# chaofengc/FeMaSR

Measured on AMD Instinct MI355X. Metric: SR output megapixels/sec at x4 (128->512), higher is better.
Workload: dtype f32 (1x1 convs / nn.Linear: every fp32 operand split EXACTLY into three bf16 terms, six partial products, fp32 accumulation on the bf16 matrix pipe - closer to fp64 than the fp32 fmaf chain, bit-identical to the CPU oracle)

## Files before the change

femasr_amd/_lib.py:

```python
import ctypes
import os

_HERE = os.path.dirname(os.path.abspath(__file__))
SO_PATH = os.path.join(_HERE, 'csrc', 'libfemasr_hip.so')

c_int, c_i64, c_f32 = ctypes.c_int, ctypes.c_int64, ctypes.c_float
vp, szt = ctypes.c_void_p, ctypes.c_size_t


class FemasrError(RuntimeError):
    pass


MAX_CODEBOOKS = 3


class Config(ctypes.Structure):
    _fields_ = ([(n, ctypes.c_int32) for n in ('in_channel', 'gt_resolution', 'lq_stage', 'scale_factor', 'use_quantize',
                                               'use_residual', 'n_codebooks')] +
                [(n, ctypes.c_int32 * MAX_CODEBOOKS) for n in ('codebook_scale', 'n_e', 'e_dim')] +
                [('device', ctypes.c_int32)])


class ConvArgs(ctypes.Structure):
    _fields_ = [
        ('in_', vp), ('B', ctypes.c_int32), ('H', ctypes.c_int32), ('W', ctypes.c_int32), ('Cin', ctypes.c_int32),
        ('w', vp), ('bias', vp),
        ('Cout', ctypes.c_int32), ('ksz', ctypes.c_int32), ('stride', ctypes.c_int32), ('pad', ctypes.c_int32),
        ('up2', ctypes.c_int32), ('prologue', ctypes.c_int32),
        ('pro_a', vp), ('pro_b', vp), ('pro_c', vp),
        ('act', ctypes.c_int32),
        ('res1', vp), ('res2', vp), ('out', vp),
        ('Ho', ctypes.c_int32), ('Wo', ctypes.c_int32),
        ('w_bf16x3', vp), ('gn_part', vp), ('w_up2', vp), ('w_wino', vp), ('fast_act', ctypes.c_int32), ('in_add', vp), ('w_bf16s', vp),
    ]


ABI_VERSION = 106
PRO_NONE, PRO_GN_SILU, PRO_LN = 0, 1, 2
ACT_NONE, ACT_GELU, ACT_RELU = 0, 1, 2

SIGNATURES = {
    'femasr_last_error': (ctypes.c_char_p, []),
    'femasr_version': (c_int, []),
    'femasr_create': (c_int, [ctypes.POINTER(Config), ctypes.POINTER(vp)]),
    'femasr_destroy': (None, [vp]),
    'femasr_num_weights': (c_int, [vp]),
    'femasr_weight_info': (c_int, [vp, c_int, ctypes.POINTER(ctypes.c_char_p), ctypes.POINTER(c_i64 * 4), ctypes.POINTER(c_int)]),
    'femasr_set_weight': (c_int, [vp, ctypes.c_char_p, vp, ctypes.POINTER(c_i64), c_int]),
    'femasr_finalize_weights': (c_int, [vp]),
    'femasr_set_streams': (c_int, [vp, c_int]),
    'femasr_workspace_bytes': (c_int, [vp, c_int, c_int, c_int, c_int, ctypes.POINTER(szt)]),
    'femasr_forward_shapes': (c_int, [vp, c_int, c_int, c_int, ctypes.POINTER(c_int), ctypes.POINTER(c_int), ctypes.POINTER(c_int),
# ... 119 lines not shown
```

femasr_amd/csrc/build.py:

```python
import os
import subprocess
import sys

HERE = os.path.dirname(os.path.abspath(__file__))
SOURCES = ['kernels_conv.hip', 'kernels_gemm.hip', 'kernels_gemm_bf16.hip', 'kernels_vq.hip', 'kernels_wino.hip', 'kernels_wino_up2.hip', 'kernels_conv_bf16.hip', 'kernels_misc.hip', 'model.hip', 'lpips.hip', 'psnr_ssim.hip', 'niqe.hip']
HEADERS = ['common.h', 'conv_common.h', 'wino_common.h', 'detmath.h', '../../include/femasr_hip.h', '../../include/femasr_hip_debug.h']
SO = os.path.join(HERE, 'libfemasr_hip.so')
FLAGS = ['--offload-arch=gfx950', '-O3', '-std=c++17', '-fPIC', '-ffp-contract=off',
         '-fhip-fp32-correctly-rounded-divide-sqrt', '-Wno-unused-result']


def _stale(target, deps):
    if not os.path.exists(target):
        return True
    t = os.path.getmtime(target)
    return any(os.path.getmtime(d) > t for d in deps)


def build(force=False, verbose=True, gate='fail'):
    hipcc = os.environ.get('HIPCC', '/opt/rocm/bin/hipcc')
    hdrs = [os.path.join(HERE, h) for h in HEADERS]
    objs, jobs = [], []
    for src in SOURCES:
        s = os.path.join(HERE, src)
# ... 9 lines not shown
        raise RuntimeError(f'hipcc failed for {failed}')
    if force or _stale(SO, objs):
        cmd = [hipcc, '--offload-arch=gfx950', '-shared', '-fPIC', '-o', SO] + objs
        if verbose:
            print(' '.join(cmd), flush=True)
        subprocess.check_call(cmd)
    if gate != 'off' and os.environ.get('FEMASR_SKIP_SCRATCH_CHECK') != '1':
        sys.path.insert(0, HERE)
        import kernel_meta
        problems = []
        try:
            _, bad = kernel_meta.check()
            if bad:
                problems.append('kernels of the default schedule use (more) scratch memory:\n' + kernel_meta.table(bad) +
                                '(fix the spill, or list the instantiation in kernel_meta.py with the reason)')
            problems += kernel_meta.check_counted_waits()
        except Exception as e:
            print(f'kernel_meta: checks skipped ({type(e).__name__}: {e})', flush=True)
        if problems and gate == 'warn':
            print('WARNING: ' + '\n'.join(problems), flush=True)
        elif problems:
            os.remove(SO)
            raise RuntimeError('\n'.join(problems))
    return SO


if __name__ == '__main__':
    build(force='--force' in sys.argv)
```

femasr_amd/csrc/common.h:

```cpp
#pragma once
#include <hip/hip_runtime.h>
#include <stdint.h>
#include <stddef.h>
#include "../../include/femasr_hip_debug.h"

int femasr_set_error(int code, const char *fmt, ...);
#define FEMASR_CHECK_HIP(expr)                                                            \
    do {                                                                                  \
        hipError_t _e = (expr);                                                           \
        if (_e != hipSuccess)                                                             \
            return femasr_set_error(FEMASR_ERR_HIP, "%s failed: %s (%s:%d)", #expr,       \
                                    hipGetErrorString(_e), __FILE__, __LINE__);           \
    } while (0)
#define FEMASR_REQUIRE(cond, ...)                                                         \
    do {                                                                                  \
        if (!(cond)) return femasr_set_error(FEMASR_ERR_INVALID, __VA_ARGS__);            \
    } while (0)

inline int femasr_allow_dynamic_lds(const void *kern, unsigned long long *devs, size_t bytes)
{
    int dev = 0;
    FEMASR_CHECK_HIP(hipGetDevice(&dev));
    if (dev < 0 || dev >= 64 || !((__atomic_load_n(devs, __ATOMIC_ACQUIRE) >> dev) & 1ull)) {
        FEMASR_CHECK_HIP(hipFuncSetAttribute(kern, hipFuncAttributeMaxDynamicSharedMemorySize, (int)bytes));
// ... 23 lines not shown
}

bool femasr_gemm_eligible(const femasr_conv_args *a);
int femasr_gemm_launch(hipStream_t s, const femasr_conv_args *a, const conv_vq_epilogue *vq, int *variant_out, double *flops_out);
int femasr_gemm_variant_count();
int femasr_gemm_pick_variant(const femasr_conv_args *a, bool vq);
const char *femasr_gemm_variant_name(int v);
int femasr_repack_k1(hipStream_t s, const float *in, int O, int I, float *out);

bool femasr_gemm_bf16s_shape_ok(const femasr_conv_args *a);
bool femasr_conv3x3_bf16s_shape_ok(const femasr_conv_args *a);
int femasr_gemm_bf16s_launch(hipStream_t s, const femasr_conv_args *a, const void *w_bf16s, int *variant_out, double *flops_out);
int femasr_gemm_bf16s_variant_count();
int femasr_gemm_bf16s_pick_variant(const femasr_conv_args *a);
const char *femasr_gemm_bf16s_variant_name(int v);

constexpr int FEMASR_WINO_LOG2_TOTAL = 31, FEMASR_WINO_LOG2_IMAGE = 27;
bool femasr_conv_wino_shape_ok(const femasr_conv_args *a);
bool femasr_conv_wino_shape_ok_lim(const femasr_conv_args *a, int log2_total, int log2_image);
int femasr_conv_wino_gn_tiles(int H, int W);
int femasr_conv_wino_launch(hipStream_t s, const femasr_conv_args *a, int *variant_out, double *flops_out);
int femasr_conv_wino_variant_count();
int femasr_conv_wino_pick_variant(const femasr_conv_args *a);
const char *femasr_conv_wino_variant_name(int v);
bool femasr_conv_wino_up2_shape_ok(const femasr_conv_args *a);
bool femasr_conv_wino_up2_shape_ok_lim(const femasr_conv_args *a, int log2_total, int log2_image);
int femasr_conv_wino_up2_launch(hipStream_t s, const femasr_conv_args *a, double *flops_out);
const char *femasr_conv_wino_up2_variant_name();

bool femasr_conv_bf16x3_eligible(const femasr_conv_args *a);
// ... 18 lines not shown
```

femasr_amd/csrc/kernel_meta.py:

```python
import os
import re
import struct
import subprocess
import sys
import tempfile

HERE = os.path.dirname(os.path.abspath(__file__))
READELF = '/opt/rocm/lib/llvm/bin/llvm-readelf'
ALLOW_SCRATCH = (
    'conv3x3_halo_bf16x3_kernel',
)


def device_elf(obj_path):
    data = open(obj_path, 'rb').read()
    i = data.find(b'__CLANG_OFFLOAD_BUNDLE__')
    if i < 0:
        return None
    n = struct.unpack_from('<Q', data, i + 24)[0]
    off = i + 32
    for _ in range(n):
        o, sz, tl = struct.unpack_from('<QQQ', data, off)
        off += 24
        triple = data[off:off + tl].decode()
# ... 69 lines not shown
            return False
        for k, lim in KNOWN_SCRATCH.items():
            if k in r['name']:
                return sz > lim
        return True
    bad = [r for r in rows if over(r)]
    if verbose:
        print(table(rows))
    return rows, bad


OBJDUMP = '/opt/rocm/lib/llvm/bin/llvm-objdump'
VMEM_PREFIXES = ('global_', 'buffer_', 'scratch_', 'flat_', 'tbuffer_')
COUNTED = {'loops': 1, 'global_load_lds_dwordx4': 12, 'global_load_dwordx4': 8, 'vmcnt': {14: 2, 10: 4}}
N_GEMM_BF16S = 9


def disassemble(obj_path):
    elf = device_elf(obj_path)
    if not elf:
        return {}
    with tempfile.NamedTemporaryFile(suffix='.co') as t:
        t.write(elf)
        t.flush()
        txt = subprocess.run([OBJDUMP, '-d', t.name], capture_output=True, text=True, check=True).stdout
    out, cur = {}, None
    for line in txt.splitlines():
        m = re.match(r'^[0-9a-f]+ <(\S+)>:', line)
        if m:
            cur = out.setdefault(m.group(1), [])
# ... 15 lines not shown
        except (ValueError, IndexError):
            continue
        if simm >= 32768:
            simm -= 65536
        if simm >= 0:
            continue
        tgt = addr_index.get(a + 4 + 4 * simm)
        if tgt is None:
            continue
        if any(o.startswith('v_mfma') for _, o, _ in insts[tgt:i]):
            loops.append((tgt, i))
    return [l for l in loops if not any(m != l and l[0] <= m[0] and m[1] <= l[1] for m in loops)]


def check_counted_waits(obj=None):
    obj = obj or os.path.join(HERE, 'kernels_gemm_bf16.o')
    problems = []
    src = open(os.path.join(HERE, 'kernels_gemm_bf16.hip')).read()
    src_counts = sorted({int(v) for v in re.findall(r's_waitcnt vmcnt\((\d+)\)', src)})
    want_counts = sorted({0} | set(COUNTED['vmcnt']))
    if src_counts != want_counts:
        problems.append(f'kernels_gemm_bf16.hip waits for vmcnt {src_counts}, kernel_meta.COUNTED expects {want_counts}: update both together')
    seen = 0
    for name, insts in disassemble(obj).items():
        if 'gemm_bf16s_kernel' not in name:
            continue
        seen += 1
        want = COUNTED
        loops = mfma_loops(insts)
        if len(loops) != want['loops']:
            problems.append(f'{demangle_short(name)}: expected {want["loops"]} MFMA loop(s), found {len(loops)}')
            continue
        for lo, hi in loops:
            body = insts[lo:hi + 1]
            vmem, waits = {}, {}
            for _, op, args in body:
                if op.startswith(VMEM_PREFIXES):
                    vmem[op] = vmem.get(op, 0) + 1
                if op == 's_waitcnt':
                    for n in re.findall(r'vmcnt\((\d+)\)', args):
                        waits[int(n)] = waits.get(int(n), 0) + 1
            want_vmem = {k: v for k, v in want.items() if k not in ('vmcnt', 'loops')}
            if vmem != want_vmem:
                problems.append(f'{demangle_short(name)}: VMEM instructions in the MFMA loop {vmem}, the counted waits assume exactly {want_vmem}')
            if waits != want['vmcnt']:
                problems.append(f'{demangle_short(name)}: vmcnt waits in the MFMA loop {waits}, the source has {want["vmcnt"]}')
            if not any(op == 's_barrier' for _, op, _ in body):
                problems.append(f'{demangle_short(name)}: no s_barrier in the MFMA loop')
    if seen < N_GEMM_BF16S:
        problems.append(f'only {seen} gemm_bf16s_kernel instantiations found in {obj}')
    return problems


META = ('vgpr_count', 'agpr_count', 'sgpr_count', 'vgpr_spill_count', 'sgpr_spill_count', 'private_segment_fixed_size', 'group_segment_fixed_size')


def code_of(csrc, objs=None):
    meta = {(r['file'], r['name']): tuple(r.get(k) for k in META) for r in kernels(csrc) if objs is None or r['file'] in objs}
    return {f: {n: ([i[1:] for i in insts], meta[f, n]) for n, insts in disassemble(os.path.join(csrc, f)).items() if (f, n) in meta}
            for f in sorted({f for f, _ in meta})}


def diff(here, there, rename=()):
    ren = dict(rename)
    lines = []
# ... 8 lines not shown
if __name__ == '__main__':
    if '--diff' in sys.argv:
        pairs = [tuple(sys.argv[i + 1].split('=', 1)) for i, a in enumerate(sys.argv) if a == '--rename']
        lines = diff(code_of(HERE), code_of(sys.argv[sys.argv.index('--diff') + 1]), pairs)
        for f, n, what in lines:
            print('%-24s %-10s %s' % (f, what, n))
        print({w: sum(1 for l in lines if l[2] == w) for w in ('same', 'differs', 'only here', 'only there')})
        sys.exit(1 if any(l[2] == 'differs' for l in lines) else 0)
    rows, bad = check(verbose='--quiet' not in sys.argv)
    if '--table' in sys.argv:
        open(sys.argv[sys.argv.index('--table') + 1], 'w').write(table(rows))
    if bad:
        print('kernels of the default schedule that use scratch memory:')
        print(table(bad))
        sys.exit(1)
    probs = check_counted_waits()
    if probs:
        print('\n'.join(probs))
        sys.exit(1)
```

femasr_amd/csrc/kernels_gemm_bf16.hip:

```cpp
#include "conv_common.h"
#include "detmath.h"
#include <stdlib.h>

typedef float f32x16 __attribute__((ext_vector_type(16)));
typedef __bf16 bf16x8 __attribute__((ext_vector_type(8)));
typedef __bf16 bf16x2_t __attribute__((ext_vector_type(2)));
typedef float f32x2_t __attribute__((ext_vector_type(2)));

namespace {

struct GemmSParams {
    const float *A;
    const uint4 *W;
    const float *bias, *res1, *res2;
    float *out;
    int M, N, K, MB, NB, NT32;
    int imH, imW, Cin, tapmul;
    int imHo, imWo, stride;
};

__device__ float g_gs_zero_page[64];

constexpr int GS_A_HALF = 3 * 2 * 128;
constexpr int GS_A_BYTES = 2 * GS_A_HALF * 16;
constexpr int GS_W_STAGE = 4 * 3 * 64;
constexpr int GS_W_STAGES = 4;
constexpr int GS_LDS_BYTES = GS_A_BYTES + GS_W_STAGES * GS_W_STAGE * 16;
static_assert(4 * TSCRATCH * 4 <= GS_LDS_BYTES, "epilogue scratch overlays the main-loop buffers");

__device__ __forceinline__ unsigned cvt_pk_bf16(float a, float b)
{
    const bf16x2_t r = __builtin_convertvector(f32x2_t{a, b}, bf16x2_t);
    return __builtin_bit_cast(unsigned, r);
}

__device__ __forceinline__ void split3_pair(float a, float b, unsigned &p1, unsigned &p2, unsigned &p3)
{
    p1 = cvt_pk_bf16(a, b);
    const float ra = a - __uint_as_float(p1 << 16), rb = b - __uint_as_float(p1 & 0xffff0000u);
    p2 = cvt_pk_bf16(ra, rb);
    const float sa = ra - __uint_as_float(p2 << 16), sb = rb - __uint_as_float(p2 & 0xffff0000u);
    p3 = cvt_pk_bf16(sa, sb);
}
__device__ __forceinline__ void split3_x8(const f32x4_t &u, const f32x4_t &v, uint4 &q1, uint4 &q2, uint4 &q3)
{
    split3_pair(u[0], u[1], q1.x, q2.x, q3.x);
    split3_pair(u[2], u[3], q1.y, q2.y, q3.y);
    split3_pair(v[0], v[1], q1.z, q2.z, q3.z);
    split3_pair(v[2], v[3], q1.w, q2.w, q3.w);
}

typedef __attribute__((address_space(3))) void *lds_vptr_s;

__device__ __forceinline__ void dma3(const uint4 *w, unsigned d0)
{
    unsigned m0_keep;
    asm volatile("s_mov_b32 %0, m0\n\t"
                 "s_mov_b32 m0, %1\n\ts_nop 0\n\tglobal_load_lds_dwordx4 %4, off\n\t"
                 "s_mov_b32 m0, %2\n\ts_nop 0\n\tglobal_load_lds_dwordx4 %5, off\n\t"
                 "s_mov_b32 m0, %3\n\ts_nop 0\n\tglobal_load_lds_dwordx4 %6, off\n\t"
                 "s_mov_b32 m0, %0"
                 : "=&s"(m0_keep) : "s"(d0), "s"(d0 + 1024u), "s"(d0 + 2048u), "v"(w), "v"(w + 64), "v"(w + 128) : "memory");
}

template <int ACT, int NRES, int CONV>
__global__ __launch_bounds__(256, 2) void gemm_bf16s_kernel(const GemmSParams p)
{
    extern __shared__ __attribute__((aligned(16))) unsigned char smem_raw[];
    uint4 *S = reinterpret_cast<uint4 *>(smem_raw);

    const int t = threadIdx.x, lane = t & 63;
    const int wave = __builtin_amdgcn_readfirstlane(t >> 6);
    const int wm = wave >> 1, wn = wave & 1;
    const int L = xcd_remap(blockIdx.x, p.MB * p.NB);
    const int nb = L % p.NB, mb = L / p.NB;
    const int m0 = mb * 128, n0 = nb * 128;
    const int h = lane >> 5, c31 = lane & 31;
    const int nsteps = p.K >> 4;
// ... 323 lines not shown
{
    const int nres = (a->res1 ? 1 : 0) + (a->res2 ? 1 : 0), act = a->act == FEMASR_ACT_GELU ? 1 : 0;
    return a->ksz == 3 ? 6 + nres : 3 * act + nres;
}

int femasr_gemm_bf16s_launch(hipStream_t s, const femasr_conv_args *a, const void *w_bf16s, int *variant_out, double *flops_out)
{
    FEMASR_REQUIRE(a && a->in && w_bf16s && femasr_gemm_bf16s_shape_ok(a), "gemm_bf16s: layer is neither a 1x1 / linear layer nor a 3x3 pad-1 conv of stride 1 or 2 with Cin %% 64 == 0");
    FEMASR_REQUIRE(a->bias && a->out, "gemm_bf16s: bias/out must be set");
    FEMASR_REQUIRE(a->act == FEMASR_ACT_NONE || a->act == FEMASR_ACT_GELU, "gemm_bf16s: bad activation %d", a->act);
    const bool conv = a->ksz == 3;
    const int Ho = conv ? (a->H - 1) / a->stride + 1 : a->H, Wo = conv ? (a->W - 1) / a->stride + 1 : a->W;
    const long long M = (long long)a->B * Ho * Wo;
    FEMASR_REQUIRE(a->Ho == Ho && a->Wo == Wo, "gemm_bf16s: Ho/Wo mismatch");
    FEMASR_REQUIRE(M > 0 && M < (1ll << 31) - 256, "gemm_bf16s: bad row count");
    GemmSParams p{};
    p.A = a->in; p.W = (const uint4 *)w_bf16s; p.bias = a->bias; p.res1 = a->res1; p.res2 = a->res2; p.out = a->out;
    p.M = (int)M; p.N = a->Cout; p.K = conv ? 9 * a->Cin : a->Cin;
    p.imH = a->H; p.imW = a->W; p.imHo = Ho; p.imWo = Wo; p.stride = a->stride; p.Cin = a->Cin; p.tapmul = ((1 << 20) + (a->Cin >> 5) - 1) / (a->Cin >> 5);
    p.NT32 = (p.N + 31) / 32;
    p.MB = (p.M + 127) / 128; p.NB = (p.N + 127) / 128;
    const int vi = femasr_gemm_bf16s_pick_variant(a);
    GSVariant &v = g_gsv[vi];
    FEMASR_CHECK(femasr_allow_dynamic_lds((const void *)v.kern, &v.attr_devs, GS_LDS_BYTES));
    hipLaunchKernelGGL(v.kern, dim3((unsigned)(p.MB * p.NB)), dim3(256), (size_t)GS_LDS_BYTES, s, p);
    FEMASR_CHECK_HIP(hipGetLastError());
    if (variant_out) *variant_out = vi;
    if (flops_out) *flops_out = 2.0 * (double)M * (double)a->Cout * (double)p.K;
    return FEMASR_OK;
}
```

femasr_amd/csrc/kernels_misc.hip:

```cpp
#include "common.h"
#include "detmath.h"
#include <stdlib.h>
#include <string.h>
#include <type_traits>

namespace {

__device__ __forceinline__ float4 ld4(const float *p) { return *reinterpret_cast<const float4 *>(p); }

__device__ __forceinline__ int xcd_remap_misc(int bid, int nblk)
{
    const int q = nblk >> 3, r = nblk & 7, xcd = bid & 7, within = bid >> 3;
    return (xcd < r ? xcd * (q + 1) : r * (q + 1) + (xcd - r) * q) + within;
}

__global__ void pad_nchw_to_nhwc_kernel(const float *__restrict__ in, int B, int C, int H, int W, int Hp, int Wp,
                                        float *__restrict__ out, size_t total)
{
    for (size_t i = blockIdx.x * (size_t)blockDim.x + threadIdx.x; i < total; i += (size_t)gridDim.x * blockDim.x) {
        const int c = (int)(i % C);
        size_t r = i / C;
        const int x = (int)(r % Wp);
        r /= Wp;
        const int y = (int)(r % Hp);
// ... 220 lines not shown
{
    const int c4n = C >> 2;
    for (size_t i = blockIdx.x * (size_t)blockDim.x + threadIdx.x; i < total4; i += (size_t)gridDim.x * blockDim.x) {
        const int c4 = (int)(i % c4n);
        const size_t n = (i / c4n) / (size_t)hw;
        const float4 v = ld4(x + 4 * i), ga = ld4(a + n * C + 4 * c4), gb = ld4(b + n * C + 4 * c4);
        float4 o;
        o.x = det_silu(__builtin_fmaf(v.x, ga.x, gb.x));
        o.y = det_silu(__builtin_fmaf(v.y, ga.y, gb.y));
        o.z = det_silu(__builtin_fmaf(v.z, ga.z, gb.z));
        o.w = det_silu(__builtin_fmaf(v.w, ga.w, gb.w));
        *reinterpret_cast<float4 *>(y + 4 * i) = o;
    }
}

__device__ __forceinline__ float wave_tree_sum(float p)
{
#pragma unroll
    for (int s = 32; s >= 1; s >>= 1) p = p + __shfl_xor(p, s, 64);
    return p;
}

__global__ void ln_stats_kernel(const float *__restrict__ x, long long rows, float eps, float *__restrict__ stats)
{
    const long long row = (long long)blockIdx.x * (blockDim.x >> 6) + (threadIdx.x >> 6);
    if (row >= rows) return;
    const int lane = threadIdx.x & 63;
    const float4 v = ld4(x + row * 256 + lane * 4);
    float s = v.x;
    s = s + v.y;
    s = s + v.z;
    s = s + v.w;
    const float mean = wave_tree_sum(s) * (1.0f / 256.0f);
    float d = v.x - mean;
    float q = d * d;
    d = v.y - mean;
    q = __builtin_fmaf(d, d, q);
    d = v.z - mean;
    q = __builtin_fmaf(d, d, q);
    d = v.w - mean;
    q = __builtin_fmaf(d, d, q);
    const float var = wave_tree_sum(q) * (1.0f / 256.0f);
    if (lane == 0) {
        stats[2 * row] = mean;
        stats[2 * row + 1] = 1.0f / sqrtf(var + eps);
    }
}

__global__ void layernorm_kernel(const float *__restrict__ x, long long rows, const float *__restrict__ gamma,
                                 const float *__restrict__ beta, float eps, float *__restrict__ y)
{
    const long long row = (long long)blockIdx.x * (blockDim.x >> 6) + (threadIdx.x >> 6);
    if (row >= rows) return;
    const int lane = threadIdx.x & 63;
    const float4 v = ld4(x + row * 256 + lane * 4);
    float s = v.x;
    s = s + v.y;
    s = s + v.z;
    s = s + v.w;
    const float mean = wave_tree_sum(s) * (1.0f / 256.0f);
    float d = v.x - mean;
    float q = d * d;
    d = v.y - mean;
    q = __builtin_fmaf(d, d, q);
    d = v.z - mean;
    q = __builtin_fmaf(d, d, q);
    d = v.w - mean;
    q = __builtin_fmaf(d, d, q);
    const float var = wave_tree_sum(q) * (1.0f / 256.0f);
    const float rstd = 1.0f / sqrtf(var + eps);
    const float4 g = ld4(gamma + lane * 4), b = ld4(beta + lane * 4);
    float4 o;
    o.x = __builtin_fmaf((v.x - mean) * rstd, g.x, b.x);
    o.y = __builtin_fmaf((v.y - mean) * rstd, g.y, b.y);
    o.z = __builtin_fmaf((v.z - mean) * rstd, g.z, b.z);
    o.w = __builtin_fmaf((v.w - mean) * rstd, g.w, b.w);
    *reinterpret_cast<float4 *>(y + row * 256 + lane * 4) = o;
}

constexpr int ATT_HD = 32, ATT_N = 64;
typedef float att_f32x16 __attribute__((ext_vector_type(16)));

template <int UNITS>
__global__ __launch_bounds__(64, 2) void window_attention_reg_kernel(const float *__restrict__ qkv, int B, int H, int W, int C,
                                                                     int heads, int shift, const float *__restrict__ table,
                                                                     float *__restrict__ out, int total)
{
    __shared__ float Ts[UNITS][232];
    const int lane = threadIdx.x, c = lane & 31, hf = lane >> 5;
    const int nwx = W >> 3, nwy = H >> 3;
    struct Unit { int h, wx, wy, n; };
    auto unit_of = [&](int bid) {
// ... 819 lines not shown

const char *femasr_conv_form_variant_name(ConvForm f, int v)
{
    switch (f) {
    case CONV_BF16X3: return femasr_conv_bf16x3_variant_name(v);
    case CONV_WINO: return femasr_conv_wino_variant_name(v);
    case CONV_WINO_UP2: return femasr_conv_wino_up2_variant_name();
    case CONV_SPLIT: return femasr_gemm_bf16s_variant_name(v);
    default: return femasr_conv_variant_name(v);
    }
}

int femasr_conv_form_launch(hipStream_t s, ConvForm f, const femasr_conv_args *a, int *slot_out, double *flops_out)
{
    int v = 0, r;
    switch (f) {
    case CONV_BF16X3: r = femasr_conv_bf16x3_launch(s, a, &v, flops_out); break;
    case CONV_WINO: r = femasr_conv_wino_launch(s, a, &v, flops_out); break;
    case CONV_WINO_UP2: r = femasr_conv_wino_up2_launch(s, a, flops_out); break;
    case CONV_SPLIT: r = femasr_gemm_bf16s_launch(s, a, a->w_bf16s, &v, flops_out); break;
    default: r = femasr_conv2d_launch(s, a, nullptr, &v, flops_out); break;
    }
    for (int g = 0; g < f; ++g) v += femasr_conv_form_variant_count((ConvForm)g);
    if (slot_out) *slot_out = v;
    return r;
}

static ConvForm conv2d_form(const femasr_conv_args *a)
{
    return !a ? CONV_DIRECT : a->w_bf16s ? CONV_SPLIT : a->w_bf16x3 ? CONV_BF16X3 : !a->w_wino ? CONV_DIRECT : a->up2 ? CONV_WINO_UP2 : CONV_WINO;
// ... 38 lines not shown
```

femasr_amd/csrc/model.hip:

```cpp
#include <stdarg.h>
#include <stdio.h>
#include <stdlib.h>
#include <string.h>

#include <algorithm>
#include <array>
#include <map>
#include <string>
#include <vector>

#include "common.h"

static thread_local char g_err[1024] = "";

int femasr_set_error(int code, const char *fmt, ...)
{
    va_list ap;
    va_start(ap, fmt);
    vsnprintf(g_err, sizeof(g_err), fmt, ap);
    va_end(ap);
    return code;
}

namespace {
// ... 763 lines not shown
    return run_tail(c, x, feats, false, false, nullptr, out_nchw, hq << h->max_depth, wq << h->max_depth);
}

int check_ready(const femasr_handle *h)
{
    FEMASR_REQUIRE(h, "null handle");
    if (!h->finalized) return femasr_set_error(FEMASR_ERR_WEIGHT, "weights not finalized: call femasr_set_weight for every key, then femasr_finalize_weights");
    return FEMASR_OK;
}

}

extern "C" {

const char *femasr_last_error(void) { return g_err; }
int femasr_version(void) { return 106; }

int femasr_create(const femasr_config *cfg, femasr_handle **out)
{
    FEMASR_REQUIRE(cfg && out, "create: null argument");
    FEMASR_REQUIRE(cfg->in_channel == 3, "create: in_channel must be 3");
    FEMASR_REQUIRE(cfg->n_codebooks >= 1 && cfg->n_codebooks <= FEMASR_MAX_CODEBOOKS, "create: n_codebooks must be 1..%d", FEMASR_MAX_CODEBOOKS);
    for (int q = 0; q < cfg->n_codebooks; ++q) {
        FEMASR_REQUIRE(cfg->n_e[q] > 0 && cfg->n_e[q] % 128 == 0 && cfg->e_dim[q] > 0 && cfg->e_dim[q] % 32 == 0,
                       "create: codebook %dx%d unsupported (n_e %% 128, e_dim %% 32)", cfg->n_e[q], cfg->e_dim[q]);
        FEMASR_REQUIRE(cfg->codebook_scale[q] > 0 && cfg->gt_resolution % cfg->codebook_scale[q] == 0, "create: bad codebook scale");
        FEMASR_REQUIRE(q == 0 || cfg->codebook_scale[q] > cfg->codebook_scale[q - 1], "create: codebook scales must ascend");
    }
    femasr_handle *h = new femasr_handle();
    h->cfg = *cfg;
    h->scale = cfg->lq_stage ? cfg->scale_factor : 1;
// ... 392 lines not shown
```

include/femasr_hip.h:

```cpp
#ifndef FEMASR_HIP_H
#define FEMASR_HIP_H

#include <stddef.h>
#include <stdint.h>

#ifdef __cplusplus
extern "C" {
#endif

typedef enum {
    FEMASR_OK = 0,
    FEMASR_ERR_INVALID = -1,
    FEMASR_ERR_HIP = -2,
    FEMASR_ERR_WEIGHT = -3,
    FEMASR_ERR_WORKSPACE = -4
} femasr_status;

typedef struct femasr_handle femasr_handle;

#define FEMASR_MAX_CODEBOOKS 3
typedef struct {
    int32_t in_channel;
    int32_t gt_resolution;
    int32_t lq_stage;
// ... 62 lines not shown
    const float *pro_a;
    const float *pro_b;
    const float *pro_c;
    int32_t act;
    const float *res1;
    const float *res2;
    float *out;
    int32_t Ho, Wo;
    const void *w_bf16x3;
    double *gn_part;
    const float *w_up2;
    const float *w_wino;
    int32_t fast_act;
    const float *in_add;
    const void *w_bf16s;
} femasr_conv_args;
int femasr_conv2d(void *stream, const femasr_conv_args *a);

size_t femasr_gn_scratch_bytes(int B, int H, int W, int C, int G);
int femasr_gn_coeffs(void *stream, const float *x, int B, int H, int W, int C, int G,
                     const float *gamma, const float *beta, float eps, float *a, float *b, void *scratch);
int femasr_gn_coeffs_from_partials(void *stream, const double *part, int B, int tiles, int H, int W, int C, int G,
                                   const float *gamma, const float *beta, float eps, float *a, float *b);
int femasr_gn_silu_apply(void *stream, const float *x, int B, int H, int W, int C, const float *a, const float *b, float *y);
int femasr_ln_stats(void *stream, const float *x, int64_t rows, int C, float eps, float *stats);
int femasr_layernorm(void *stream, const float *x, int64_t rows, int C, const float *gamma, const float *beta,
                     float eps, float *y);
int femasr_window_attention(void *stream, const float *qkv, int B, int H, int W, int C, int heads, int shift,
                            const float *table, float *out);
int femasr_vq(void *stream, const float *z, int64_t M, int D, const float *cb, const float *cbT,
// ... 84 lines not shown
```

Measured before the change: 67.91.

## Add row-owning 1x1 Cout=256 bf16x3 GEMM kernel with optional fused LayerNorm output

Adds a new GEMM kernel for 1x1 layers with 256 output channels and no activation. Each 64-row block computes all 256 columns, so a whole output row lives in one block and the epilogue can apply bias and residuals and optionally write a LayerNorm of the row. The existing bf16s launcher now routes eligible layers to this kernel. This is meant to get better A-tile reuse and to open the door to fusing the following LayerNorm. The model code shown never sets ln_out, so the LN fusion is plumbing only. The new kernel uses a smaller M tile, so the block count and occupancy trade-offs change.

```diff
diff --git a/femasr_amd/_lib.py b/femasr_amd/_lib.py
--- a/femasr_amd/_lib.py
+++ b/femasr_amd/_lib.py
@@ -33,10 +33,11 @@
         ('res1', vp), ('res2', vp), ('out', vp),
         ('Ho', ctypes.c_int32), ('Wo', ctypes.c_int32),
         ('w_bf16x3', vp), ('gn_part', vp), ('w_up2', vp), ('w_wino', vp), ('fast_act', ctypes.c_int32), ('in_add', vp), ('w_bf16s', vp),
+        ('ln_gamma', vp), ('ln_beta', vp), ('ln_eps', c_f32), ('ln_out', vp),
     ]
 
 
-ABI_VERSION = 106
+ABI_VERSION = 107
 PRO_NONE, PRO_GN_SILU, PRO_LN = 0, 1, 2
 ACT_NONE, ACT_GELU, ACT_RELU = 0, 1, 2
 
diff --git a/femasr_amd/csrc/build.py b/femasr_amd/csrc/build.py
--- a/femasr_amd/csrc/build.py
+++ b/femasr_amd/csrc/build.py
@@ -3,8 +3,8 @@
 import sys
 
 HERE = os.path.dirname(os.path.abspath(__file__))
-SOURCES = ['kernels_conv.hip', 'kernels_gemm.hip', 'kernels_gemm_bf16.hip', 'kernels_vq.hip', 'kernels_wino.hip', 'kernels_wino_up2.hip', 'kernels_conv_bf16.hip', 'kernels_misc.hip', 'model.hip', 'lpips.hip', 'psnr_ssim.hip', 'niqe.hip']
-HEADERS = ['common.h', 'conv_common.h', 'wino_common.h', 'detmath.h', '../../include/femasr_hip.h', '../../include/femasr_hip_debug.h']
+SOURCES = ['kernels_conv.hip', 'kernels_gemm.hip', 'kernels_gemm_bf16.hip', 'kernels_gemm_bf16_rows.hip', 'kernels_vq.hip', 'kernels_wino.hip', 'kernels_wino_up2.hip', 'kernels_conv_bf16.hip', 'kernels_misc.hip', 'model.hip', 'lpips.hip', 'psnr_ssim.hip', 'niqe.hip']
+HEADERS = ['common.h', 'conv_common.h', 'wino_common.h', 'detmath.h', 'split_bf16.h', 'layernorm_row.h', '../../include/femasr_hip.h', '../../include/femasr_hip_debug.h']
 SO = os.path.join(HERE, 'libfemasr_hip.so')
 FLAGS = ['--offload-arch=gfx950', '-O3', '-std=c++17', '-fPIC', '-ffp-contract=off',
          '-fhip-fp32-correctly-rounded-divide-sqrt', '-Wno-unused-result']
@@ -47,7 +47,7 @@
             if bad:
                 problems.append('kernels of the default schedule use (more) scratch memory:\n' + kernel_meta.table(bad) +
                                 '(fix the spill, or list the instantiation in kernel_meta.py with the reason)')
-            problems += kernel_meta.check_counted_waits()
+            problems += kernel_meta.check_counted_waits() + kernel_meta.check_counted_waits_rows()
         except Exception as e:
             print(f'kernel_meta: checks skipped ({type(e).__name__}: {e})', flush=True)
         if problems and gate == 'warn':
diff --git a/femasr_amd/csrc/common.h b/femasr_amd/csrc/common.h
--- a/femasr_amd/csrc/common.h
+++ b/femasr_amd/csrc/common.h
@@ -61,6 +61,8 @@
 int femasr_gemm_bf16s_variant_count();
 int femasr_gemm_bf16s_pick_variant(const femasr_conv_args *a);
 const char *femasr_gemm_bf16s_variant_name(int v);
+bool femasr_gemm_rows_takes(const femasr_conv_args *a);
+int femasr_gemm_rows_launch(hipStream_t s, const femasr_conv_args *a, const void *w_bf16s, long long M);
 
 constexpr int FEMASR_WINO_LOG2_TOTAL = 31, FEMASR_WINO_LOG2_IMAGE = 27;
 bool femasr_conv_wino_shape_ok(const femasr_conv_args *a);
diff --git a/femasr_amd/csrc/kernel_meta.py b/femasr_amd/csrc/kernel_meta.py
--- a/femasr_amd/csrc/kernel_meta.py
+++ b/femasr_amd/csrc/kernel_meta.py
@@ -107,6 +107,8 @@
 VMEM_PREFIXES = ('global_', 'buffer_', 'scratch_', 'flat_', 'tbuffer_')
 COUNTED = {'loops': 1, 'global_load_lds_dwordx4': 12, 'global_load_dwordx4': 8, 'vmcnt': {14: 2, 10: 4}}
 N_GEMM_BF16S = 9
+COUNTED_ROWS = {'loops': 1, 'global_load_lds_dwordx4': 24, 'global_load_dwordx4': 4, 'vmcnt': {8: 4, 14: 2}}
+N_GEMM_ROWS = 3
 
 
 def disassemble(obj_path):
@@ -152,19 +154,26 @@
 
 
 def check_counted_waits(obj=None):
-    obj = obj or os.path.join(HERE, 'kernels_gemm_bf16.o')
+    return _check_counted(obj or os.path.join(HERE, 'kernels_gemm_bf16.o'), 'kernels_gemm_bf16.hip', 'gemm_bf16s_kernel', COUNTED, 'COUNTED', N_GEMM_BF16S)
+
+
+def check_counted_waits_rows(obj=None):
+    return _check_counted(obj or os.path.join(HERE, 'kernels_gemm_bf16_rows.o'), 'kernels_gemm_bf16_rows.hip', 'linear_rows256_kernel', COUNTED_ROWS,
+                          'COUNTED_ROWS', N_GEMM_ROWS)
+
+
+def _check_counted(obj, source, kernel, want, want_name, n_inst):
     problems = []
-    src = open(os.path.join(HERE, 'kernels_gemm_bf16.hip')).read()
+    src = open(os.path.join(HERE, source)).read()
     src_counts = sorted({int(v) for v in re.findall(r's_waitcnt vmcnt\((\d+)\)', src)})
-    want_counts = sorted({0} | set(COUNTED['vmcnt']))
+    want_counts = sorted({0} | set(want['vmcnt']))
     if src_counts != want_counts:
-        problems.append(f'kernels_gemm_bf16.hip waits for vmcnt {src_counts}, kernel_meta.COUNTED expects {want_counts}: update both together')
+        problems.append(f'{source} waits for vmcnt {src_counts}, kernel_meta.{want_name} expects {want_counts}: update both together')
     seen = 0
     for name, insts in disassemble(obj).items():
-        if 'gemm_bf16s_kernel' not in name:
+        if kernel not in name:
             continue
         seen += 1
-        want = COUNTED
         loops = mfma_loops(insts)
         if len(loops) != want['loops']:
             problems.append(f'{demangle_short(name)}: expected {want["loops"]} MFMA loop(s), found {len(loops)}')
@@ -185,8 +194,8 @@
                 problems.append(f'{demangle_short(name)}: vmcnt waits in the MFMA loop {waits}, the source has {want["vmcnt"]}')
             if not any(op == 's_barrier' for _, op, _ in body):
                 problems.append(f'{demangle_short(name)}: no s_barrier in the MFMA loop')
-    if seen < N_GEMM_BF16S:
-        problems.append(f'only {seen} gemm_bf16s_kernel instantiations found in {obj}')
+    if seen < n_inst:
+        problems.append(f'only {seen} {kernel} instantiations found in {obj}')
     return problems
 
 
@@ -225,7 +234,7 @@
         print('kernels of the default schedule that use scratch memory:')
         print(table(bad))
         sys.exit(1)
-    probs = check_counted_waits()
+    probs = check_counted_waits() + check_counted_waits_rows()
     if probs:
         print('\n'.join(probs))
         sys.exit(1)
diff --git a/femasr_amd/csrc/kernels_gemm_bf16.hip b/femasr_amd/csrc/kernels_gemm_bf16.hip
--- a/femasr_amd/csrc/kernels_gemm_bf16.hip
+++ b/femasr_amd/csrc/kernels_gemm_bf16.hip
@@ -1,11 +1,6 @@
-#include "conv_common.h"
+#include "split_bf16.h"
 #include "detmath.h"
 #include <stdlib.h>
-
-typedef float f32x16 __attribute__((ext_vector_type(16)));
-typedef __bf16 bf16x8 __attribute__((ext_vector_type(8)));
-typedef __bf16 bf16x2_t __attribute__((ext_vector_type(2)));
-typedef float f32x2_t __attribute__((ext_vector_type(2)));
 
 namespace {
 
@@ -27,41 +22,6 @@
 constexpr int GS_W_STAGES = 4;
 constexpr int GS_LDS_BYTES = GS_A_BYTES + GS_W_STAGES * GS_W_STAGE * 16;
 static_assert(4 * TSCRATCH * 4 <= GS_LDS_BYTES, "epilogue scratch overlays the main-loop buffers");
-
-__device__ __forceinline__ unsigned cvt_pk_bf16(float a, float b)
-{
-    const bf16x2_t r = __builtin_convertvector(f32x2_t{a, b}, bf16x2_t);
-    return __builtin_bit_cast(unsigned, r);
-}
-
-__device__ __forceinline__ void split3_pair(float a, float b, unsigned &p1, unsigned &p2, unsigned &p3)
-{
-    p1 = cvt_pk_bf16(a, b);
-    const float ra = a - __uint_as_float(p1 << 16), rb = b - __uint_as_float(p1 & 0xffff0000u);
-    p2 = cvt_pk_bf16(ra, rb);
-    const float sa = ra - __uint_as_float(p2 << 16), sb = rb - __uint_as_float(p2 & 0xffff0000u);
-    p3 = cvt_pk_bf16(sa, sb);
-}
-__device__ __forceinline__ void split3_x8(const f32x4_t &u, const f32x4_t &v, uint4 &q1, uint4 &q2, uint4 &q3)
-{
-    split3_pair(u[0], u[1], q1.x, q2.x, q3.x);
-    split3_pair(u[2], u[3], q1.y, q2.y, q3.y);
-    split3_pair(v[0], v[1], q1.z, q2.z, q3.z);
-    split3_pair(v[2], v[3], q1.w, q2.w, q3.w);
-}
-
-typedef __attribute__((address_space(3))) void *lds_vptr_s;
-
-__device__ __forceinline__ void dma3(const uint4 *w, unsigned d0)
-{
-    unsigned m0_keep;
-    asm volatile("s_mov_b32 %0, m0\n\t"
-                 "s_mov_b32 m0, %1\n\ts_nop 0\n\tglobal_load_lds_dwordx4 %4, off\n\t"
-                 "s_mov_b32 m0, %2\n\ts_nop 0\n\tglobal_load_lds_dwordx4 %5, off\n\t"
-                 "s_mov_b32 m0, %3\n\ts_nop 0\n\tglobal_load_lds_dwordx4 %6, off\n\t"
-                 "s_mov_b32 m0, %0"
-                 : "=&s"(m0_keep) : "s"(d0), "s"(d0 + 1024u), "s"(d0 + 2048u), "v"(w), "v"(w + 64), "v"(w + 128) : "memory");
-}
 
 template <int ACT, int NRES, int CONV>
 __global__ __launch_bounds__(256, 2) void gemm_bf16s_kernel(const GemmSParams p)
@@ -415,18 +375,20 @@
     const long long M = (long long)a->B * Ho * Wo;
     FEMASR_REQUIRE(a->Ho == Ho && a->Wo == Wo, "gemm_bf16s: Ho/Wo mismatch");
     FEMASR_REQUIRE(M > 0 && M < (1ll << 31) - 256, "gemm_bf16s: bad row count");
+    const int vi = femasr_gemm_bf16s_pick_variant(a);
+    if (variant_out) *variant_out = vi;
+    if (flops_out) *flops_out = 2.0 * (double)M * (double)a->Cout * (double)(conv ? 9 * a->Cin : a->Cin);
+    if (femasr_gemm_rows_takes(a)) return femasr_gemm_rows_launch(s, a, w_bf16s, M);
+    FEMASR_REQUIRE(!a->ln_out, "gemm_bf16s: ln_out is only written by the row-owning form (1x1, Cout = 256, no activation)");
     GemmSParams p{};
     p.A = a->in; p.W = (const uint4 *)w_bf16s; p.bias = a->bias; p.res1 = a->res1; p.res2 = a->res2; p.out = a->out;
     p.M = (int)M; p.N = a->Cout; p.K = conv ? 9 * a->Cin : a->Cin;
     p.imH = a->H; p.imW = a->W; p.imHo = Ho; p.imWo = Wo; p.stride = a->stride; p.Cin = a->Cin; p.tapmul = ((1 << 20) + (a->Cin >> 5) - 1) / (a->Cin >> 5);
     p.NT32 = (p.N + 31) / 32;
     p.MB = (p.M + 127) / 128; p.NB = (p.N + 127) / 128;
-    const int vi = femasr_gemm_bf16s_pick_variant(a);
     GSVariant &v = g_gsv[vi];
     FEMASR_CHECK(femasr_allow_dynamic_lds((const void *)v.kern, &v.attr_devs, GS_LDS_BYTES));
     hipLaunchKernelGGL(v.kern, dim3((unsigned)(p.MB * p.NB)), dim3(256), (size_t)GS_LDS_BYTES, s, p);
     FEMASR_CHECK_HIP(hipGetLastError());
-    if (variant_out) *variant_out = vi;
-    if (flops_out) *flops_out = 2.0 * (double)M * (double)a->Cout * (double)p.K;
     return FEMASR_OK;
 }
diff --git a/femasr_amd/csrc/kernels_gemm_bf16_rows.hip b/femasr_amd/csrc/kernels_gemm_bf16_rows.hip
--- /dev/null
+++ b/femasr_amd/csrc/kernels_gemm_bf16_rows.hip
@@ -0,0 +1,223 @@
+#include "split_bf16.h"
+#include "layernorm_row.h"
+#include <stdlib.h>
+
+namespace {
+
+struct RowsParams {
+    const float *A;
+    const uint4 *W;
+    const float *bias, *res1, *res2;
+    float *out;
+    const float *ln_gamma, *ln_beta;
+    float *ln_out;
+    float ln_eps;
+    int M, K, MB;
+};
+
+constexpr int GR_A_HALF = 3 * 2 * 64;
+constexpr int GR_A_CHUNK = 2 * GR_A_HALF;
+constexpr int GR_A_BYTES = 2 * GR_A_CHUNK * 16;
+constexpr int GR_W_STAGE = 8 * 3 * 64;
+constexpr int GR_W_STAGES = 2;
+constexpr int GR_LDS_BYTES = GR_A_BYTES + GR_W_STAGES * GR_W_STAGE * 16;
+constexpr int GR_PITCH = 264;
+static_assert(64 * GR_PITCH * 4 <= GR_LDS_BYTES, "the epilogue row tile overlays the main-loop buffers");
+static_assert(2 * GR_LDS_BYTES <= 160 * 1024, "two blocks per CU");
+
+template <int NRES>
+__global__ __launch_bounds__(256, 2) void linear_rows256_kernel(const RowsParams p)
+{
+    extern __shared__ __attribute__((aligned(16))) unsigned char smem_raw[];
+    uint4 *Al = reinterpret_cast<uint4 *>(smem_raw);
+    uint4 *Wl = reinterpret_cast<uint4 *>(smem_raw + GR_A_BYTES);
+
+    const int t = threadIdx.x, lane = t & 63;
+    const int wave = __builtin_amdgcn_readfirstlane(t >> 6);
+    const int m0 = xcd_remap(blockIdx.x, p.MB) * 64;
+    const int h = lane >> 5, c31 = lane & 31;
+    const int nsteps = p.K >> 4, nch = p.K >> 5;
+
+    const uint4 *srcW = p.W + wave * 384 + lane;
+    const unsigned lds0 = __builtin_amdgcn_readfirstlane((unsigned)(size_t)(lds_vptr_s)Al);
+    const unsigned ldsW = lds0 + (unsigned)GR_A_BYTES + (unsigned)wave * 6144u;
+    auto issueW = [&](int s) {
+        const uint4 *w = srcW + (size_t)(s < nsteps ? s : nsteps - 1) * GR_W_STAGE;
+        const unsigned d = ldsW + (unsigned)(s & 1) * (GR_W_STAGE * 16);
+        dma3(w, d);
+        dma3(w + 192, d + 3072u);
+    };
+
+    const int q = t & 3, srow = t >> 2;
+    int grow = m0 + srow;
+    grow = grow < p.M ? grow : p.M - 1;
+    const float *srcA = p.A + (size_t)grow * p.K + 8 * q;
+    const int dstA = (q >> 1) * GR_A_HALF + (q & 1) * 64 + ((srow + 4 * (q & 1) + 8 * (q >> 1)) & 63);
+    f32x4_t ar[2][2] = {};
+    auto loadA = [&](int c, f32x4_t (&r)[2]) {
+        const float *g = srcA + (c < nch ? c : nch - 1) * 32;
+        asm volatile("global_load_dwordx4 %0, %2, off\n\tglobal_load_dwordx4 %1, %2, off offset:16"
+                     : "=&v"(r[0]), "=&v"(r[1]) : "v"(g) : "memory");
+    };
+    auto splitA = [&](const f32x4_t (&r)[2], int buf) {
+        uint4 q1, q2, q3;
+        split3_x8(r[0], r[1], q1, q2, q3);
+        uint4 *d = Al + buf * GR_A_CHUNK + dstA;
+        d[0] = q1;
+        d[128] = q2;
+        d[256] = q3;
+    };
+    int aoff[2][2];
+#pragma unroll
+    for (int st = 0; st < 2; ++st)
+#pragma unroll
+        for (int rt = 0; rt < 2; ++rt) aoff[st][rt] = st * GR_A_HALF + h * 64 + ((rt * 32 + c31 + 4 * h + 8 * st) & 63);
+    const int boff = wave * 384 + lane;
+
+    f32x16 hi[2][2], lo[2][2];
+#pragma unroll
+    for (int i = 0; i < 2; ++i)
+#pragma unroll
+        for (int j = 0; j < 2; ++j)
+#pragma unroll
+            for (int r = 0; r < 16; ++r) { hi[i][j][r] = 0.f; lo[i][j][r] = 0.f; }
+
+    auto step = [&](int s, int buf, int st, auto &&between) {
+        const uint4 *As = Al + buf * GR_A_CHUNK, *Ws = Wl + st * GR_W_STAGE + boff;
+        bf16x8 fa[3][2], fb[3][2];
+#pragma unroll
+        for (int pl = 0; pl < 3; ++pl) {
+#pragma unroll
+            for (int rt = 0; rt < 2; ++rt) fa[pl][rt] = __builtin_bit_cast(bf16x8, As[pl * 128 + aoff[st][rt]]);
+#pragma unroll
+            for (int ct = 0; ct < 2; ++ct) fb[pl][ct] = __builtin_bit_cast(bf16x8, Ws[ct * 192 + pl * 64]);
+        }
+        asm volatile("s_waitcnt lgkmcnt(0)" ::: "memory");
+        issueW(s + 2);
+        between();
+#define GR_TERM(ACC, PA, PB)                                                                                       \
+    _Pragma("unroll") for (int rt = 0; rt < 2; ++rt)                                                              \
+        _Pragma("unroll") for (int ct = 0; ct < 2; ++ct)                                                          \
+            ACC[rt][ct] = __builtin_amdgcn_mfma_f32_32x32x16_bf16(fa[PA][rt], fb[PB][ct], ACC[rt][ct], 0, 0, 0);
+        GR_TERM(lo, 2, 0)
+        GR_TERM(lo, 0, 2)
+        GR_TERM(lo, 1, 1)
+        GR_TERM(lo, 1, 0)
+        GR_TERM(lo, 0, 1)
+        GR_TERM(hi, 0, 0)
+#undef GR_TERM
+    };
+
+    loadA(0, ar[0]);
+    issueW(0);
+    loadA(1, ar[1]);
+    issueW(1);
+    asm volatile("s_waitcnt vmcnt(14)" : "+v"(ar[0][0]), "+v"(ar[0][1]) :: "memory");
+    splitA(ar[0], 0);
+
+    auto chunk = [&](int c, int buf, f32x4_t (&cur)[2], f32x4_t (&nxt)[2]) {
+        asm volatile("s_waitcnt vmcnt(8)\n\ts_waitcnt lgkmcnt(0)" ::: "memory");
+        __builtin_amdgcn_s_barrier();
+        asm volatile("" ::: "memory");
+        step(2 * c, buf, 0, [&] {
+            loadA(c + 2, cur);
+            asm volatile("s_waitcnt vmcnt(14)" : "+v"(nxt[0]), "+v"(nxt[1]) :: "memory");
+            splitA(nxt, buf ^ 1);
+        });
+        asm volatile("s_waitcnt vmcnt(8)" ::: "memory");
+        step(2 * c + 1, buf, 1, [] {});
+    };
+#pragma unroll 1
+    for (int c = 0; c < nch; c += 2) {
+        chunk(c, 0, ar[0], ar[1]);
+        chunk(c + 1, 1, ar[1], ar[0]);
+    }
+
+    asm volatile("s_waitcnt vmcnt(0)" ::: "memory");
+    float *R = reinterpret_cast<float *>(smem_raw);
+    const float *ra = p.res1 ? p.res1 : p.res2, *rb = (p.res1 && p.res2) ? p.res2 : nullptr;
+    const bool ln = p.ln_out != nullptr;
+    constexpr int BR = 8;
+    const int lrow0 = wave * 16;
+    float4 r1[2][BR] = {}, r2[2][BR] = {};
+    auto fetch_res = [&](int b, float4 (&d1)[BR], float4 (&d2)[BR]) {
+        if (NRES == 0) return;
+#pragma unroll
+        for (int k = 0; k < BR; ++k) {
+            int row = m0 + lrow0 + b * BR + k;
+            row = row < p.M ? row : p.M - 1;
+            d1[k] = ld4(ra + (size_t)row * 256 + 4 * lane);
+            if (NRES >= 2) d2[k] = ld4(rb + (size_t)row * 256 + 4 * lane);
+        }
+    };
+    const float4 b4 = ld4(p.bias + 4 * lane);
+    float4 g4 = {0.f, 0.f, 0.f, 0.f}, be4 = {0.f, 0.f, 0.f, 0.f};
+    if (ln) { g4 = ld4(p.ln_gamma + 4 * lane); be4 = ld4(p.ln_beta + 4 * lane); }
+    fetch_res(0, r1[0], r2[0]);
+    asm volatile("s_waitcnt lgkmcnt(0)" ::: "memory");
+    __builtin_amdgcn_s_barrier();
+    asm volatile("" ::: "memory");
+#pragma unroll
+    for (int i = 0; i < 2; ++i)
+#pragma unroll
+        for (int j = 0; j < 2; ++j)
+#pragma unroll
+            for (int r = 0; r < 16; ++r)
+                R[(i * 32 + (r & 3) + 8 * (r >> 2) + 4 * h) * GR_PITCH + wave * 64 + j * 32 + c31] = hi[i][j][r] + lo[i][j][r];
+    asm volatile("s_waitcnt lgkmcnt(0)" ::: "memory");
+    __builtin_amdgcn_s_barrier();
+    asm volatile("" ::: "memory");
+#pragma unroll
+    for (int b = 0; b < 16 / BR; ++b) {
+        if (b + 1 < 16 / BR) fetch_res(b + 1, r1[(b + 1) & 1], r2[(b + 1) & 1]);
+        float4 v[BR], n[BR];
+#pragma unroll
+        for (int k = 0; k < BR; ++k) {
+            const float4 a4 = *reinterpret_cast<const float4 *>(R + (lrow0 + b * BR + k) * GR_PITCH + 4 * lane);
+            v[k] = float4{a4.x + b4.x, a4.y + b4.y, a4.z + b4.z, a4.w + b4.w};
+            if (NRES >= 1) { const float4 &e = r1[b & 1][k]; v[k].x = v[k].x + e.x; v[k].y = v[k].y + e.y; v[k].z = v[k].z + e.z; v[k].w = v[k].w + e.w; }
+            if (NRES >= 2) { const float4 &e = r2[b & 1][k]; v[k].x = v[k].x + e.x; v[k].y = v[k].y + e.y; v[k].z = v[k].z + e.z; v[k].w = v[k].w + e.w; }
+        }
+        if (ln) {
+#pragma unroll
+            for (int k = 0; k < BR; ++k) n[k] = ln_row256(v[k], g4, be4, p.ln_eps);
+        }
+#pragma unroll
+        for (int k = 0; k < BR; ++k) {
+            const int row = m0 + lrow0 + b * BR + k;
+            if (row < p.M) {
+                *reinterpret_cast<float4 *>(p.out + (size_t)row * 256 + 4 * lane) = v[k];
+                if (ln) *reinterpret_cast<float4 *>(p.ln_out + (size_t)row * 256 + 4 * lane) = n[k];
+            }
+        }
+    }
+}
+
+struct RowsVariant {
+    void (*kern)(const RowsParams);
+    unsigned long long attr_devs;
+};
+RowsVariant g_rows[3] = { { linear_rows256_kernel<0>, 0ull }, { linear_rows256_kernel<1>, 0ull }, { linear_rows256_kernel<2>, 0ull } };
+
+}
+
+bool femasr_gemm_rows_takes(const femasr_conv_args *a)
+{
+    return a->ksz == 1 && a->pad == 0 && a->stride == 1 && !a->up2 && a->Cout == 256 && a->Cin > 0 && (a->Cin % 64) == 0 &&
+           a->prologue == FEMASR_PRO_NONE && a->act == FEMASR_ACT_NONE;
+}
+
+int femasr_gemm_rows_launch(hipStream_t s, const femasr_conv_args *a, const void *w_bf16s, long long M)
+{
+    FEMASR_REQUIRE(femasr_gemm_rows_takes(a), "gemm_rows: not a 1x1 layer with 256 output channels and no activation");
+    FEMASR_REQUIRE(!a->ln_out || (a->ln_gamma && a->ln_beta), "gemm_rows: ln_out needs ln_gamma and ln_beta");
+    RowsParams p{};
+    p.A = a->in; p.W = (const uint4 *)w_bf16s; p.bias = a->bias; p.res1 = a->res1; p.res2 = a->res2; p.out = a->out;
+    p.ln_gamma = a->ln_gamma; p.ln_beta = a->ln_beta; p.ln_out = a->ln_out; p.ln_eps = a->ln_eps;
+    p.M = (int)M; p.K = a->Cin; p.MB = (p.M + 63) / 64;
+    RowsVariant &v = g_rows[(a->res1 ? 1 : 0) + (a->res2 ? 1 : 0)];
+    FEMASR_CHECK(femasr_allow_dynamic_lds((const void *)v.kern, &v.attr_devs, GR_LDS_BYTES));
+    hipLaunchKernelGGL(v.kern, dim3((unsigned)p.MB), dim3(256), (size_t)GR_LDS_BYTES, s, p);
+    FEMASR_CHECK_HIP(hipGetLastError());
+    return FEMASR_OK;
+}
diff --git a/femasr_amd/csrc/kernels_misc.hip b/femasr_amd/csrc/kernels_misc.hip
--- a/femasr_amd/csrc/kernels_misc.hip
+++ b/femasr_amd/csrc/kernels_misc.hip
@@ -1,5 +1,6 @@
 #include "common.h"
 #include "detmath.h"
+#include "layernorm_row.h"
 #include <stdlib.h>
 #include <string.h>
 #include <type_traits>
@@ -258,36 +259,17 @@
     }
 }
 
-__device__ __forceinline__ float wave_tree_sum(float p)
-{
-#pragma unroll
-    for (int s = 32; s >= 1; s >>= 1) p = p + __shfl_xor(p, s, 64);
-    return p;
-}
-
 __global__ void ln_stats_kernel(const float *__restrict__ x, long long rows, float eps, float *__restrict__ stats)
 {
     const long long row = (long long)blockIdx.x * (blockDim.x >> 6) + (threadIdx.x >> 6);
     if (row >= rows) return;
     const int lane = threadIdx.x & 63;
     const float4 v = ld4(x + row * 256 + lane * 4);
-    float s = v.x;
-    s = s + v.y;
-    s = s + v.z;
-    s = s + v.w;
-    const float mean = wave_tree_sum(s) * (1.0f / 256.0f);
-    float d = v.x - mean;
-    float q = d * d;
-    d = v.y - mean;
-    q = __builtin_fmaf(d, d, q);
-    d = v.z - mean;
-    q = __builtin_fmaf(d, d, q);
-    d = v.w - mean;
-    q = __builtin_fmaf(d, d, q);
-    const float var = wave_tree_sum(q) * (1.0f / 256.0f);
+    float mean, rstd;
+    ln_row256_moments(v, eps, mean, rstd);
     if (lane == 0) {
         stats[2 * row] = mean;
-        stats[2 * row + 1] = 1.0f / sqrtf(var + eps);
+        stats[2 * row + 1] = rstd;
     }
 }
 
@@ -298,28 +280,7 @@
     if (row >= rows) return;
     const int lane = threadIdx.x & 63;
     const float4 v = ld4(x + row * 256 + lane * 4);
-    float s = v.x;
-    s = s + v.y;
-    s = s + v.z;
-    s = s + v.w;
-    const float mean = wave_tree_sum(s) * (1.0f / 256.0f);
-    float d = v.x - mean;
-    float q = d * d;
-    d = v.y - mean;
-    q = __builtin_fmaf(d, d, q);
-    d = v.z - mean;
-    q = __builtin_fmaf(d, d, q);
-    d = v.w - mean;
-    q = __builtin_fmaf(d, d, q);
-    const float var = wave_tree_sum(q) * (1.0f / 256.0f);
-    const float rstd = 1.0f / sqrtf(var + eps);
-    const float4 g = ld4(gamma + lane * 4), b = ld4(beta + lane * 4);
-    float4 o;
-    o.x = __builtin_fmaf((v.x - mean) * rstd, g.x, b.x);
-    o.y = __builtin_fmaf((v.y - mean) * rstd, g.y, b.y);
-    o.z = __builtin_fmaf((v.z - mean) * rstd, g.z, b.z);
-    o.w = __builtin_fmaf((v.w - mean) * rstd, g.w, b.w);
-    *reinterpret_cast<float4 *>(y + row * 256 + lane * 4) = o;
+    *reinterpret_cast<float4 *>(y + row * 256 + lane * 4) = ln_row256(v, ld4(gamma + lane * 4), ld4(beta + lane * 4), eps);
 }
 
 constexpr int ATT_HD = 32, ATT_N = 64;
@@ -1169,6 +1130,15 @@
 int femasr_conv_form_launch(hipStream_t s, ConvForm f, const femasr_conv_args *a, int *slot_out, double *flops_out)
 {
     int v = 0, r;
+    if (a && a->ln_out) {
+        FEMASR_REQUIRE(f == CONV_SPLIT && a->w_bf16s && femasr_gemm_rows_takes(a),
+                       "conv2d: ln_out is only written by a 1x1 stride-1 w_bf16s layer with Cout = 256, Cin %% 64 == 0, no prologue, no activation");
+        FEMASR_REQUIRE(a->ln_gamma && a->ln_beta, "conv2d: ln_out needs ln_gamma and ln_beta");
+        const size_t nout = (size_t)a->B * a->Ho * a->Wo * a->Cout, nin = (size_t)a->B * a->H * a->W * a->Cin;
+        auto overlaps = [&](const float *q, size_t n) { return q && q < a->ln_out + nout && a->ln_out < q + n; };
+        FEMASR_REQUIRE(!overlaps(a->in, nin) && !overlaps(a->res1, nout) && !overlaps(a->res2, nout) && !overlaps(a->out, nout),
+                       "conv2d: ln_out overlaps in / res1 / res2 / out");
+    }
     switch (f) {
     case CONV_BF16X3: r = femasr_conv_bf16x3_launch(s, a, &v, flops_out); break;
     case CONV_WINO: r = femasr_conv_wino_launch(s, a, &v, flops_out); break;
diff --git a/femasr_amd/csrc/layernorm_row.h b/femasr_amd/csrc/layernorm_row.h
--- /dev/null
+++ b/femasr_amd/csrc/layernorm_row.h
@@ -0,0 +1,44 @@
+#pragma once
+#include <hip/hip_runtime.h>
+
+namespace {
+
+__device__ __forceinline__ float wave_tree_sum(float p)
+{
+#pragma unroll
+    for (int s = 32; s >= 1; s >>= 1) p = p + __shfl_xor(p, s, 64);
+    return p;
+}
+
+__device__ __forceinline__ void ln_row256_moments(const float4 &v, float eps, float &mean, float &rstd)
+{
+    float s = v.x;
+    s = s + v.y;
+    s = s + v.z;
+    s = s + v.w;
+    mean = wave_tree_sum(s) * (1.0f / 256.0f);
+    float d = v.x - mean;
+    float q = d * d;
+    d = v.y - mean;
+    q = __builtin_fmaf(d, d, q);
+    d = v.z - mean;
+    q = __builtin_fmaf(d, d, q);
+    d = v.w - mean;
+    q = __builtin_fmaf(d, d, q);
+    const float var = wave_tree_sum(q) * (1.0f / 256.0f);
+    rstd = 1.0f / sqrtf(var + eps);
+}
+
+__device__ __forceinline__ float4 ln_row256(const float4 &v, const float4 &g, const float4 &b, float eps)
+{
+    float mean, rstd;
+    ln_row256_moments(v, eps, mean, rstd);
+    float4 o;
+    o.x = __builtin_fmaf((v.x - mean) * rstd, g.x, b.x);
+    o.y = __builtin_fmaf((v.y - mean) * rstd, g.y, b.y);
+    o.z = __builtin_fmaf((v.z - mean) * rstd, g.z, b.z);
+    o.w = __builtin_fmaf((v.w - mean) * rstd, g.w, b.w);
+    return o;
+}
+
+}
diff --git a/femasr_amd/csrc/model.hip b/femasr_amd/csrc/model.hip
--- a/femasr_amd/csrc/model.hip
+++ b/femasr_amd/csrc/model.hip
@@ -801,7 +801,7 @@
 extern "C" {
 
 const char *femasr_last_error(void) { return g_err; }
-int femasr_version(void) { return 106; }
+int femasr_version(void) { return 107; }
 
 int femasr_create(const femasr_config *cfg, femasr_handle **out)
 {
diff --git a/femasr_amd/csrc/split_bf16.h b/femasr_amd/csrc/split_bf16.h
--- /dev/null
+++ b/femasr_amd/csrc/split_bf16.h
@@ -0,0 +1,46 @@
+#pragma once
+#include "conv_common.h"
+
+typedef float f32x16 __attribute__((ext_vector_type(16)));
+typedef __bf16 bf16x8 __attribute__((ext_vector_type(8)));
+typedef __bf16 bf16x2_t __attribute__((ext_vector_type(2)));
+typedef float f32x2_t __attribute__((ext_vector_type(2)));
+
+namespace {
+
+__device__ __forceinline__ unsigned cvt_pk_bf16(float a, float b)
+{
+    const bf16x2_t r = __builtin_convertvector(f32x2_t{a, b}, bf16x2_t);
+    return __builtin_bit_cast(unsigned, r);
+}
+
+__device__ __forceinline__ void split3_pair(float a, float b, unsigned &p1, unsigned &p2, unsigned &p3)
+{
+    p1 = cvt_pk_bf16(a, b);
+    const float ra = a - __uint_as_float(p1 << 16), rb = b - __uint_as_float(p1 & 0xffff0000u);
+    p2 = cvt_pk_bf16(ra, rb);
+    const float sa = ra - __uint_as_float(p2 << 16), sb = rb - __uint_as_float(p2 & 0xffff0000u);
+    p3 = cvt_pk_bf16(sa, sb);
+}
+__device__ __forceinline__ void split3_x8(const f32x4_t &u, const f32x4_t &v, uint4 &q1, uint4 &q2, uint4 &q3)
+{
+    split3_pair(u[0], u[1], q1.x, q2.x, q3.x);
+    split3_pair(u[2], u[3], q1.y, q2.y, q3.y);
+    split3_pair(v[0], v[1], q1.z, q2.z, q3.z);
+    split3_pair(v[2], v[3], q1.w, q2.w, q3.w);
+}
+
+typedef __attribute__((address_space(3))) void *lds_vptr_s;
+
+__device__ __forceinline__ void dma3(const uint4 *w, unsigned d0)
+{
+    unsigned m0_keep;
+    asm volatile("s_mov_b32 %0, m0\n\t"
+                 "s_mov_b32 m0, %1\n\ts_nop 0\n\tglobal_load_lds_dwordx4 %4, off\n\t"
+                 "s_mov_b32 m0, %2\n\ts_nop 0\n\tglobal_load_lds_dwordx4 %5, off\n\t"
+                 "s_mov_b32 m0, %3\n\ts_nop 0\n\tglobal_load_lds_dwordx4 %6, off\n\t"
+                 "s_mov_b32 m0, %0"
+                 : "=&s"(m0_keep) : "s"(d0), "s"(d0 + 1024u), "s"(d0 + 2048u), "v"(w), "v"(w + 64), "v"(w + 128) : "memory");
+}
+
+}
diff --git a/include/femasr_hip.h b/include/femasr_hip.h
--- a/include/femasr_hip.h
+++ b/include/femasr_hip.h
@@ -100,6 +100,10 @@
     int32_t fast_act;
     const float *in_add;
     const void *w_bf16s;
+    const float *ln_gamma;
+    const float *ln_beta;
+    float ln_eps;
+    float *ln_out;
 } femasr_conv_args;
 int femasr_conv2d(void *stream, const femasr_conv_args *a);
 
```

After: 68.03 (median of 2 runs). Within noise of the previous version (+0.2%).
